# tfzhou/ContrastiveSeg

Hardware: AMD Instinct MI355X
Metric: images/sec contrastive train step, HRNet-W48 1024x512 bs8 (higher is better)
Workload: dtype fp32 in/out, f16x3 split MFMA (fp32 accumulate); 1 GPU; cfg2: BASELINE.json configs[1]: HRNet-W48 + contrast_ce_loss, synthetic Cityscapes 3x512x1024x19, tau=0.1, max_samples=1024, with_embed=True, SGD(0.01,0.9,5; model=hrnet_w48_contrast, loss=contrast_ce_loss, global_batch=8, per_gpu_batch=8, arithmetic=f16x3 on the matrix cores for the 3x3 / 1x1 convolutions, rest fp32, parallelism=dp1, step_graph=eager (auto: per-GPU batch above 1, the GPU is the limit)

## Files before the change

contrastiveseg_amd/_hip.py:

```python
import ctypes
import os

import torch

_PKG = os.path.dirname(os.path.abspath(__file__))
LIB_PATH = os.path.join(_PKG, "libcseg_hip.so")

_c_int = ctypes.c_int
_c_float = ctypes.c_float
_ptr = ctypes.c_void_p


class ContrastDesc(ctypes.Structure):
    _fields_ = [("mode", _c_int), ("N", _c_int), ("M", _c_int), ("D", _c_int),
                ("anchors", _ptr), ("a_lab", _ptr), ("contrast", _ptr), ("c_lab", _ptr),
                ("segment_queue", _ptr), ("pixel_queue", _ptr),
                ("bank_classes", _c_int), ("bank_size", _c_int),
                ("temperature", _c_float), ("base_temperature", _c_float)]


class ConvGroupMember(ctypes.Structure):
    _fields_ = [("x", _ptr), ("wp", _ptr), ("bias", _ptr), ("addend", _ptr), ("y", _ptr), ("stats", _ptr), ("amax_x", _ptr),
                ("amax_w", _ptr), ("B", _c_int), ("Cin", _c_int), ("Cout", _c_int), ("H", _c_int), ("W", _c_int),
                ("reserved", _c_int * 3)]
# ... 59 lines not shown
    "cseg_conv1x1_sb_packed_bytes": (ctypes.c_size_t, [_c_int, _c_int]),
    "cseg_conv1x1_sb_pack_weights": (_c_int, [_ptr, _c_int, _c_int, _c_int, _ptr, _ptr]),
    "cseg_conv1x1_sb_fwd": (_c_int, [_ptr, _ptr, _ptr, _c_int, _c_int, _c_int, _c_int, _ptr, _ptr]),
    "cseg_conv1x1_sb_wrw_ws_floats": (ctypes.c_size_t, [_c_int] * 4),
    "cseg_conv1x1_sb_wrw": (_c_int, [_ptr, _ptr, _c_int, _c_int, _c_int, _c_int, _ptr, _ptr, _ptr]),
    "cseg_amax_f32": (_c_int, [_ptr, ctypes.c_long, _ptr, _ptr]),
    "cseg_conv3x3_split_packed_bytes": (ctypes.c_size_t, [_c_int, _c_int, _c_int]),
    "cseg_conv3x3_split_pack": (_c_int, [_ptr, _c_int, _c_int, _c_int, _c_int, _c_int, _ptr, _ptr, _ptr]),
    "cseg_conv3x3_split_fwd": (_c_int, [_ptr, _ptr, _ptr] + [_c_int] * 7 + [_ptr, _ptr, _ptr, _ptr]),
    "cseg_conv3x3_split_wrw": (_c_int, [_ptr, _ptr] + [_c_int] * 6 + [_ptr, _ptr, _ptr, _ptr, _ptr]),
    "cseg_conv3x3_split_fwd_add": (_c_int, [_ptr, _ptr, _ptr, _ptr] + [_c_int] * 7 + [_ptr, _ptr, _ptr, _ptr]),
    "cseg_conv3x3_split_group_fwd": (_c_int, [_ptr, _c_int, _c_int, _ptr, _ptr]),
    "cseg_conv3x3_split_group_wrw": (_c_int, [_ptr, _c_int, _c_int, _ptr]),
    "cseg_bn_group_tiles_finalize": (_c_int, [_ptr, _c_int, _ptr]),
    "cseg_bn_group_apply": (_c_int, [_ptr, _c_int, _c_int, _ptr]),
    "cseg_bn_group_bwd": (_c_int, [_ptr, _c_int, _c_int, _c_int, _ptr]),
    "cseg_bn_group_tiles_moments": (_c_int, [_ptr, _c_int, _ptr, _ptr]),
    "cseg_bn_group_finalize": (_c_int, [_ptr, _c_int, _ptr, _ptr]),
    "cseg_bn_group_bwd_reduce": (_c_int, [_ptr, _c_int, _c_int, _ptr, _ptr]),
    "cseg_bn_group_bwd_apply": (_c_int, [_ptr, _c_int, _c_int, _ptr, _ptr]),
    "cseg_conv3x3_split_dil_fwd": (_c_int, [_ptr, _ptr, _ptr, _ptr] + [_c_int] * 7 + [_ptr, _ptr, _ptr, _ptr, _ptr]),
    "cseg_conv3x3_s2_split_packed_bytes": (ctypes.c_size_t, [_c_int] * 2),
    "cseg_conv3x3_s2_split_plan": (_c_int, [_c_int] * 4 + [_ptr, _ptr]),
    "cseg_conv3x3_s2_split_pack": (_c_int, [_ptr] + [_c_int] * 4 + [_ptr, _ptr, _ptr]),
    "cseg_conv3x3_s2_split_fwd": (_c_int, [_ptr, _ptr] + [_c_int] * 6 + [_ptr, _ptr, _ptr, _ptr]),
    "cseg_conv3x3_s2_split_bwd": (_c_int, [_ptr, _ptr] + [_c_int] * 6 + [_ptr, _ptr, _ptr, _ptr]),
    "cseg_conv3x3_s2_rgb_fwd": (_c_int, [_ptr, _ptr] + [_c_int] * 4 + [_ptr, _ptr]),
    "cseg_conv3x3_s2_rgb_wrw_ws_floats": (ctypes.c_size_t, [_c_int] * 4),
    "cseg_conv3x3_s2_rgb_wrw": (_c_int, [_ptr, _ptr] + [_c_int] * 4 + [_ptr, _ptr, _ptr]),
    "cseg_cls1x1_fwd": (_c_int, [_ptr, _ptr, _ptr] + [_c_int] * 4 + [ctypes.c_long, _ptr, _ptr]),
    "cseg_cls1x1_bwd": (_c_int, [_ptr, _ptr] + [_c_int] * 4 + [ctypes.c_long, _ptr, _ptr]),
    "cseg_cls1x1_wrw_ws_floats": (ctypes.c_size_t, [_c_int, _c_int, _c_int, ctypes.c_long]),
    "cseg_cls1x1_wrw": (_c_int, [_ptr, _ptr] + [_c_int] * 4 + [ctypes.c_long, _ptr, _ptr, _ptr]),
    "cseg_conv3x3_s2_wrw_ws_floats": (ctypes.c_size_t, [_c_int] * 5),
    "cseg_conv3x3_s2_split_wrw": (_c_int, [_ptr, _ptr] + [_c_int] * 6 + [_ptr, _ptr, _ptr, _ptr, _ptr]),
    "cseg_conv1x1_split_packed_bytes": (ctypes.c_size_t, [_c_int, _c_int, _c_int]),
    "cseg_conv1x1_split_pack": (_c_int, [_ptr, _c_int, _c_int, _c_int, _c_int, _ptr, _ptr, _ptr]),
    "cseg_conv1x1_split_fwd": (_c_int, [_ptr, _ptr, _ptr] + [_c_int] * 5 + [_ptr, _ptr, _ptr, _ptr]),
    "cseg_conv1x1_split_fwd_add": (_c_int, [_ptr, _ptr, _ptr, _ptr] + [_c_int] * 5 + [_ptr, _ptr, _ptr, _ptr]),
    "cseg_conv1x1_split_wrw": (_c_int, [_ptr, _ptr] + [_c_int] * 5 + [_ptr, _ptr, _ptr, _ptr, _ptr]),
    "cseg_conv3x3_split_plan": (_c_int, [_c_int, _c_int, _c_int, _ptr, _ptr, _ptr]),
    "cseg_conv1x1_split_plan": (_c_int, [_c_int, _c_int, _ptr, _ptr]),
    "cseg_conv1x1_split_plan_arith": (_c_int, [_c_int, _c_int, _c_int, ctypes.POINTER(_c_int), ctypes.POINTER(ctypes.c_long)]),
    "cseg_amax_batch": (_c_int, [_ptr, _c_int, _c_int, _ptr]),
    "cseg_split_pack_batch": (_c_int, [_ptr, _c_int, _c_int, _c_int, _ptr]),
    "cseg_augment_batch": (_c_int, [_ptr, _ptr, _ptr, _ptr] + [_c_int] * 5 + [_c_float, _ptr, _ptr, _ptr, _ptr, _ptr]),
    "cseg_conv_stat_segments": (ctypes.c_size_t, [_c_int] * 4),
    "cseg_conv3x3_split_fwd_st": (_c_int, [_ptr, _ptr, _ptr] + [_c_int] * 7 + [_ptr, _ptr, _ptr, _ptr, _ptr]),
    "cseg_conv1x1_split_fwd_st": (_c_int, [_ptr, _ptr, _ptr] + [_c_int] * 5 + [_ptr, _ptr, _ptr, _ptr, _ptr]),
    "cseg_conv3x3_s2_split_fwd_st": (_c_int, [_ptr, _ptr] + [_c_int] * 6 + [_ptr, _ptr, _ptr, _ptr, _ptr]),
    "cseg_bn_tiles_finalize": (_c_int, [_ptr, _c_int, ctypes.c_long, _c_float, _c_float, _ptr, _ptr, _ptr, _ptr, _ptr]),
    "cseg_bn_tiles_moments": (_c_int, [_ptr, _c_int, ctypes.c_long, _ptr, _ptr]),
    "cseg_bn_ws_floats": (ctypes.c_size_t, [_c_int, _c_int, _c_int]),
    "cseg_bn_stats": (_c_int, [_ptr, _c_int, _c_int, _c_int, _ptr, _ptr, _ptr]),
    "cseg_bn_finalize": (_c_int, [_ptr, _c_int, ctypes.c_double, _c_float, _c_float, _ptr, _ptr, _ptr, _ptr, _ptr]),
    "cseg_bn_stats_finalize": (_c_int, [_ptr, _c_int, _c_int, _c_int, _ptr, _c_float, _c_float, _ptr, _ptr, _ptr, _ptr,
                                        _ptr]),
    "cseg_bn_fwd": (_c_int, [_ptr] * 4 + [_c_int] * 4 + [_ptr, _c_float, _c_float] + [_ptr] * 5 + [_ptr]),
    "cseg_bn_bwd": (_c_int, [_ptr] * 6 + [_c_int] * 5 + [_ptr] * 5 + [_ptr]),
    "cseg_bn_fwd_amax": (_c_int, [_ptr] * 4 + [_c_int] * 4 + [_ptr, _c_float, _c_float] + [_ptr] * 5 + [_ptr, _ptr]),
    "cseg_bn_bwd_amax": (_c_int, [_ptr] * 6 + [_c_int] * 5 + [_ptr] * 5 + [_ptr, _ptr]),
    "cseg_bn_apply_amax": (_c_int, [_ptr, _ptr, _ptr, _ptr, _ptr, _c_int, _c_int, _c_int, _c_int, _ptr, _ptr, _ptr]),
    "cseg_bn_bwd_apply_amax": (_c_int, [_ptr] * 6 + [ctypes.c_double, _c_int, _c_int, _c_int, _c_int, _ptr, _ptr, _ptr]),
    "cseg_bn_apply": (_c_int, [_ptr, _ptr, _ptr, _ptr, _ptr, _c_int, _c_int, _c_int, _c_int, _ptr, _ptr]),
    "cseg_bn_bwd_reduce": (_c_int, [_ptr] * 6 + [_c_int] * 4 + [_ptr] * 5 + [_ptr]),
    "cseg_bn_bwd_apply": (_c_int, [_ptr] * 6 + [ctypes.c_double, _c_int, _c_int, _c_int, _c_int, _ptr, _ptr]),
# ... 54 lines not shown
```

contrastiveseg_amd/csrc/cls1x1.hip:

```cpp
#include "cseg_common.h"
#include "cseg_hip.h"

namespace {

constexpr int PX = 128;

template <int KP>
__global__ __launch_bounds__(256) void cls1x1_fwd_kernel(const float* __restrict__ x, const float* __restrict__ wt,
                                                         const float* __restrict__ bias, int C, int K, long P, int tiles,
                                                         float* __restrict__ y) {
    __shared__ float red[PX][KP + 1];
    const int b = blockIdx.x / tiles, tile = blockIdx.x - b * tiles;
    const int half = __builtin_amdgcn_readfirstlane((int)threadIdx.x / PX), lp = threadIdx.x - half * PX;
    const long p = (long)tile * PX + lp;
    const bool live = p < P;
    const long pc = live ? p : P - 1;
    const int c_mid = (C + 1) / 2;
    const int c0 = half ? c_mid : 0, c1 = half ? C : c_mid;
    const float* xp = x + ((size_t)b * C + c0) * P + pc;
    const float* wp = wt + ((size_t)b * C + c0) * KP;
    float acc[KP];
#pragma unroll
    for (int k = 0; k < KP; ++k) acc[k] = 0.f;
    int c = c0;
    for (; c + 8 <= c1; c += 8) {
        float v[8];
#pragma unroll
        for (int j = 0; j < 8; ++j) v[j] = xp[(size_t)j * P];
#pragma unroll
        for (int j = 0; j < 8; ++j)
#pragma unroll
            for (int k = 0; k < KP; ++k) acc[k] = __builtin_fmaf(v[j], wp[j * KP + k], acc[k]);
        xp += (size_t)8 * P;
        wp += 8 * KP;
    }
    for (; c < c1; ++c) {
        const float v = xp[0];
#pragma unroll
        for (int k = 0; k < KP; ++k) acc[k] = __builtin_fmaf(v, wp[k], acc[k]);
        xp += P;
        wp += KP;
    }
    if (half) {
#pragma unroll
        for (int k = 0; k < KP; ++k) red[lp][k] = acc[k];
    }
    __syncthreads();
    if (!half && live) {
        float* yp = y + (size_t)b * K * P + p;
#pragma unroll
        for (int k = 0; k < KP; ++k)
            if (k < K) yp[(size_t)k * P] = (acc[k] + red[lp][k]) + (bias ? bias[k] : 0.f);
    }
}

template <int KP, bool VEC>
__global__ __launch_bounds__(256) void cls1x1_bwd_kernel(const float* __restrict__ dy, const float* __restrict__ wt, int C, int K,
                                                         long P, int tiles, float* __restrict__ dx) {
    constexpr int V = VEC ? 4 : 1;
    const int b = blockIdx.x / tiles, tile = blockIdx.x - b * tiles;
    const long p = ((long)tile * 256 + threadIdx.x) * V;
    const bool live = p < P;
    const long pc = live ? p : 0;
    float d[KP][V];
#pragma unroll
    for (int k = 0; k < KP; ++k) {
        if (k < K) {
            const float* src = dy + ((size_t)b * K + k) * P + pc;
            if (VEC) {
                const float4 t4 = *reinterpret_cast<const float4*>(src);
                d[k][0] = t4.x; d[k][1 % V] = t4.y; d[k][2 % V] = t4.z; d[k][3 % V] = t4.w;
            } else {
                d[k][0] = *src;
            }
        } else {
#pragma unroll
            for (int t = 0; t < V; ++t) d[k][t] = 0.f;
        }
    }
    const int per = (C + (int)gridDim.y - 1) / (int)gridDim.y;
    const int c0 = blockIdx.y * per, c1 = min(C, c0 + per);
    const float* wp = wt + ((size_t)b * C + c0) * KP;
    float* op = dx + ((size_t)b * C + c0) * P + pc;
    for (int c = c0; c < c1; ++c) {
        float s[V];
#pragma unroll
        for (int t = 0; t < V; ++t) s[t] = 0.f;
#pragma unroll
        for (int k = 0; k < KP; ++k)
#pragma unroll
            for (int t = 0; t < V; ++t) s[t] = __builtin_fmaf(wp[k], d[k][t], s[t]);
        if (live) {
            if (VEC) *reinterpret_cast<float4*>(op) = make_float4(s[0], s[1 % V], s[2 % V], s[3 % V]);
            else *op = s[0];
        }
        wp += KP;
        op += P;
    }
}

constexpr int WC = 64, WP = 64;
constexpr int A_PITCH = WP + 1;

template <int KP, bool VEC>
__global__ __launch_bounds__(256) void cls1x1_wrw_kernel(const float* __restrict__ x, const float* __restrict__ dy, int C, int K, long P,
                                                         int c_tiles, int n_split, float* __restrict__ partial) {
    __shared__ __attribute__((aligned(16))) float As[WC * A_PITCH];
    __shared__ __attribute__((aligned(16))) float Ds[WP * KP];
    __shared__ float red[3][WC][KP + 1];
    int blk = blockIdx.x;
    const int split = blk % n_split; blk /= n_split;
    const int ct = blk % c_tiles;
    const int b = blk / c_tiles;
    const int tid = threadIdx.x, wave = tid >> 6, lane = tid & 63;
    const long stages = (P + WP - 1) / WP;
    const long s0 = stages * split / n_split, s1 = stages * (split + 1) / n_split;
    const int cb = ct * WC;
    float acc[KP];
#pragma unroll
    for (int k = 0; k < KP; ++k) acc[k] = 0.f;
    const int a_ch = tid >> 2, a_px = (tid & 3) * 16;
    const bool a_ok = cb + a_ch < C;
    const float* a_src = x + ((size_t)b * C + min(cb + a_ch, C - 1)) * P;
    const int d_k = tid >> 4, d_px = (tid & 15) * 4;
    for (long st = s0; st < s1; ++st) {
        const long p0 = st * WP;
        float av[16], dv0[4], dv1[4];
        if (VEC && p0 + WP <= P) {
#pragma unroll
            for (int q = 0; q < 4; ++q) {
                const float4 t4 = *reinterpret_cast<const float4*>(a_src + p0 + a_px + 4 * q);
                av[4 * q] = t4.x; av[4 * q + 1] = t4.y; av[4 * q + 2] = t4.z; av[4 * q + 3] = t4.w;
            }
        } else {
#pragma unroll
            for (int j = 0; j < 16; ++j) av[j] = p0 + a_px + j < P ? a_src[p0 + a_px + j] : 0.f;
        }
#pragma unroll
        for (int j = 0; j < 4; ++j) {
            const long p = p0 + d_px + j;
            dv0[j] = (d_k < K && p < P) ? dy[((size_t)b * K + d_k) * P + p] : 0.f;
            dv1[j] = (d_k + 16 < K && p < P) ? dy[((size_t)b * K + d_k + 16) * P + p] : 0.f;
        }
        __syncthreads();
#pragma unroll
        for (int j = 0; j < 16; ++j) As[a_ch * A_PITCH + a_px + j] = a_ok ? av[j] : 0.f;
#pragma unroll
        for (int j = 0; j < 4; ++j) {
            Ds[(d_px + j) * KP + d_k] = dv0[j];
            if (d_k + 16 < KP) Ds[(d_px + j) * KP + d_k + 16] = dv1[j];
        }
        __syncthreads();
#pragma unroll 4
        for (int j = 0; j < WP / 4; ++j) {
            const int p = wave * (WP / 4) + j;
            const float a = As[lane * A_PITCH + p];
#pragma unroll
            for (int k4 = 0; k4 < KP / 4; ++k4) {
                const float4 d4 = *reinterpret_cast<const float4*>(Ds + p * KP + 4 * k4);
                acc[4 * k4] = __builtin_fmaf(a, d4.x, acc[4 * k4]);
                acc[4 * k4 + 1] = __builtin_fmaf(a, d4.y, acc[4 * k4 + 1]);
                acc[4 * k4 + 2] = __builtin_fmaf(a, d4.z, acc[4 * k4 + 2]);
                acc[4 * k4 + 3] = __builtin_fmaf(a, d4.w, acc[4 * k4 + 3]);
            }
        }
    }
    if (wave > 0) {
#pragma unroll
        for (int k = 0; k < KP; ++k) red[wave - 1][lane][k] = acc[k];
    }
    __syncthreads();
    if (wave == 0 && cb + lane < C) {
        const int B = gridDim.x / (n_split * c_tiles);
        float* out = partial + (((size_t)split * B + b) * C + (cb + lane)) * KP;
#pragma unroll
        for (int k = 0; k < KP; ++k) out[k] = ((acc[k] + red[0][lane][k]) + red[1][lane][k]) + red[2][lane][k];
    }
}

__global__ __launch_bounds__(256) void cls1x1_wrw_reduce_kernel(const float* __restrict__ partial, int n_split, long total,
                                                                float* __restrict__ dwt) {
    const long e = (long)blockIdx.x * 256 + threadIdx.x;
    if (e >= total) return;
    float s = 0.f;
    for (int sp = 0; sp < n_split; ++sp) s += partial[(size_t)sp * total + e];
    dwt[e] = s;
}

int wrw_splits(int B, int C, long P) {
    const long stages = (P + WP - 1) / WP;
    const long groups = (long)B * ((C + WC - 1) / WC);
    long n = (1536 + groups - 1) / groups;
    if (n > stages) n = stages;
    if (n > 64) n = 64;
    return (int)(n < 1 ? 1 : n);
}

bool shape_ok(int B, int C, int K, int KP, long P) {
    return B > 0 && C > 0 && K > 0 && K <= KP && (KP == 20 || KP == 32) && P > 0 && (long)B * C * P < (1L << 40) &&
           (long)B * ((P + PX - 1) / PX) < 2147483647L / 16;
}

}

extern "C" int cseg_cls1x1_fwd(const float* x, const float* wt, const float* bias, int B, int C, int K, int KP, long P, float* y,
                               cseg_stream_t stream_) {
    CSEG_REQUIRE(x && wt && y, "cls1x1_fwd: null pointer");
    CSEG_REQUIRE(shape_ok(B, C, K, KP, P), "cls1x1_fwd: unsupported shape B=%d C=%d K=%d KP=%d P=%ld (K <= KP, KP 20 or 32)", B, C, K, KP, P);
    hipStream_t stream = (hipStream_t)stream_;
    const int tiles = (int)((P + PX - 1) / PX);
    if (KP == 20)
        hipLaunchKernelGGL(cls1x1_fwd_kernel<20>, dim3((unsigned)(B * tiles)), dim3(256), 0, stream, x, wt, bias, C, K, P, tiles, y);
    else
        hipLaunchKernelGGL(cls1x1_fwd_kernel<32>, dim3((unsigned)(B * tiles)), dim3(256), 0, stream, x, wt, bias, C, K, P, tiles, y);
    CSEG_CHECK_LAUNCH("cls1x1_fwd_kernel");
    return 1;
}

extern "C" int cseg_cls1x1_bwd(const float* dy, const float* wt, int B, int C, int K, int KP, long P, float* dx, cseg_stream_t stream_) {
    CSEG_REQUIRE(dy && wt && dx, "cls1x1_bwd: null pointer");
    CSEG_REQUIRE(shape_ok(B, C, K, KP, P), "cls1x1_bwd: unsupported shape B=%d C=%d K=%d KP=%d P=%ld (K <= KP, KP 20 or 32)", B, C, K, KP, P);
    hipStream_t stream = (hipStream_t)stream_;
    const bool vec = P % 4 == 0 && ((reinterpret_cast<uintptr_t>(dy) | reinterpret_cast<uintptr_t>(dx)) & 15) == 0;
    const long per_block = vec ? 1024 : 256;
    const int tiles = (int)((P + per_block - 1) / per_block);
    int parts = 1;
    while (parts < 16 && (long)B * tiles * parts < 2048 && C / (parts * 2) >= 32) parts *= 2;
#define CLS_BWD(KPV, V)                                                                                                                \
    hipLaunchKernelGGL((cls1x1_bwd_kernel<KPV, V>), dim3((unsigned)(B * tiles), parts), dim3(256), 0, stream, dy, wt, C, K, P, tiles, dx)
    if (KP == 20) { if (vec) CLS_BWD(20, true); else CLS_BWD(20, false); }
    else          { if (vec) CLS_BWD(32, true); else CLS_BWD(32, false); }
#undef CLS_BWD
    CSEG_CHECK_LAUNCH("cls1x1_bwd_kernel");
    return 1;
}

extern "C" size_t cseg_cls1x1_wrw_ws_floats(int B, int C, int KP, long P) {
    if (B <= 0 || C <= 0 || P <= 0 || (KP != 20 && KP != 32)) return 0;
    return (size_t)wrw_splits(B, C, P) * B * C * KP;
}

extern "C" int cseg_cls1x1_wrw(const float* x, const float* dy, int B, int C, int K, int KP, long P, float* ws, float* dwt,
                               cseg_stream_t stream_) {
    CSEG_REQUIRE(x && dy && ws && dwt, "cls1x1_wrw: null pointer");
    CSEG_REQUIRE(shape_ok(B, C, K, KP, P), "cls1x1_wrw: unsupported shape B=%d C=%d K=%d KP=%d P=%ld (K <= KP, KP 20 or 32)", B, C, K, KP, P);
    hipStream_t stream = (hipStream_t)stream_;
    const int n_split = wrw_splits(B, C, P), c_tiles = (C + WC - 1) / WC;
    const long blocks = (long)B * c_tiles * n_split;
    CSEG_REQUIRE(blocks < 2147483647L, "cls1x1_wrw: grid too large");
    const bool vec = P % 4 == 0 && (reinterpret_cast<uintptr_t>(x) & 15) == 0;
#define CLS_WRW(KPV, V)                                                                                                            \
    hipLaunchKernelGGL((cls1x1_wrw_kernel<KPV, V>), dim3((unsigned)blocks), dim3(256), 0, stream, x, dy, C, K, P, c_tiles, n_split, ws)
    if (KP == 20) { if (vec) CLS_WRW(20, true); else CLS_WRW(20, false); }
    else          { if (vec) CLS_WRW(32, true); else CLS_WRW(32, false); }
#undef CLS_WRW
    CSEG_CHECK_LAUNCH("cls1x1_wrw_kernel");
    const long total = (long)B * C * KP;
    hipLaunchKernelGGL(cls1x1_wrw_reduce_kernel, dim3((unsigned)((total + 255) / 256)), dim3(256), 0, stream, ws, n_split, total, dwt);
    CSEG_CHECK_LAUNCH("cls1x1_wrw_reduce_kernel");
    return 1;
}
```

contrastiveseg_amd/kernels.py:

```python
import ctypes

import os

import torch
from torch.autograd import Function

from . import _hip

I32, I16, I64, F32 = torch.int32, torch.int16, torch.int64, torch.float32


def _p(t, dtype, what):
    return _hip.dev(t, dtype, what)


def _null():
    return ctypes.c_void_p(None)


def _on_device(t):
    return t.is_cuda


def _pq(t, what):
# ... 1826 lines not shown
        K_, KP, P = ctx.K, wt.shape[2], H * W
        dx = dwt = db = None
        if ctx.needs_input_grad[0]:
            dx = torch.empty_like(x)
            _hip.call("cseg_cls1x1_bwd", _p(dy, F32, "dy"), _p(wt, F32, "wt"), B, C, K_, KP, ctypes.c_long(P), _pf(dx), _hip.stream_ptr())
        if ctx.needs_input_grad[1]:
            n = _hip.lib().cseg_cls1x1_wrw_ws_floats(B, C, KP, ctypes.c_long(P))
            if n == 0:
                raise RuntimeError("cls1x1_wrw: unsupported shape %s x %s" % (tuple(x.shape), tuple(dy.shape)))
            ws = torch.empty(n, dtype=F32, device=x.device)
            dwt = torch.empty(B, C, KP, dtype=F32, device=x.device)
            _hip.call("cseg_cls1x1_wrw", _p(x, F32, "x"), _p(dy, F32, "dy"), B, C, K_, KP, ctypes.c_long(P), _pf(ws), _pf(dwt),
                      _hip.stream_ptr())
        if ctx.has_bias and ctx.needs_input_grad[2]:
            db = dy.sum((0, 2, 3))
        return dx, dwt, db, None


def cls1x1_weights(weight, B, mask=None):
    K_, C = weight.shape[:2]
    KP = cls1x1_kp(K_)
    w2 = weight.reshape(K_, C).t()
    if KP > K_:
        w2 = torch.nn.functional.pad(w2, (0, KP - K_))
    if mask is None:
        return w2.unsqueeze(0).expand(B, C, KP).contiguous()
    return w2.unsqueeze(0) * mask.reshape(B, C, 1)


def cls1x1(x, weight, bias=None, mask=None):
    return Cls1x1.apply(x, cls1x1_weights(weight, x.shape[0], mask), bias, weight.shape[0])


CONV1X1_SPLIT_BF16 = os.environ.get("CSEG_CONV1X1_SPLIT_BF16", "1") == "1"
CONV1X1_SB_MIN_TILES = int(os.environ.get("CSEG_SB_MIN_TILES", "1"))


def conv1x1_sb_eligible(x, weight):
    if not (_on_device(x) and x.dtype == F32 and weight.dtype == F32 and x.dim() == 4 and x.is_contiguous()):
        return False
    co, ci, kh, kw = weight.shape
    ok = lambda c: c % 48 == 0 or c % 64 == 0
    return (kh, kw) == (1, 1) and ok(ci) and ok(co) and x.shape[1] == ci


def conv1x1_sb_tiles(x, c_out):
    nt16 = next(16 * nt for nt in (9, 8, 6, 4, 3) if c_out % (16 * nt) == 0)
    return x.shape[0] * (c_out // nt16) * ((x.shape[2] * x.shape[3] + 255) // 256)


def conv1x1_sb_pack(weight, transpose=False):
    return SPLIT_WEIGHTS.get(weight, "c1", transpose, 0)


def conv1x1_sb_run(x, weight, transpose=False, bias=None, ax=None, want_stats=False, addend=None):
    co, ci = weight.shape[:2]
    conv_in, conv_out = (co, ci) if transpose else (ci, co)
    B, _, H, W = x.shape
    arith = split_arith_id()
    wp, aw = conv1x1_sb_pack(weight, transpose)
    if arith and ax is None:
        ax = tensor_amax(x)
    y = torch.empty(B, conv_out, H, W, dtype=F32, device=x.device)
    if want_stats and CONV_EPILOGUE_STATS:
        st = tile_stats_buffer(1, conv_out, B, H * W, 1, x.device)
        _hip.call("cseg_conv1x1_split_fwd_st", _pq(x, "x"), wp.data_ptr(), _opt(bias, F32, "bias"), B, conv_in, conv_out, H * W,
# ... 168 lines not shown
```

contrastiveseg_amd/lib/models/nets/hrnet.py:

```python
import torch
import torch.nn as nn

from contrastiveseg_amd import kernels as K
from contrastiveseg_amd.lib.models.backbones.backbone_selector import BackboneSelector
from contrastiveseg_amd.lib.models.modules.projection import ProjectionHead
from contrastiveseg_amd.lib.models.modules.spatial_ocr_block import SpatialGather_Module, SpatialOCR_Module
from contrastiveseg_amd.lib.models.tools.module_helper import (ClassifierConv1x1, FoldedDropout2d, HeadConv3x3, ModuleHelper,
                                                                  SplitConv2d)


import os as _os

_HEAD_STREAMS = {}
HEAD_FORK = _os.environ.get("CSEG_HEAD_FORK", "0") == "1"


def _fork_heads(feats):
    from contrastiveseg_amd.lib.models.backbones import hrnet_backbone as HB
    if not (HEAD_FORK and feats.is_cuda and HB.EAGER_FORKS and torch.is_grad_enabled()) or torch.cuda.is_current_stream_capturing():
        return None
    key = feats.device.index
    if key not in _HEAD_STREAMS:
        _HEAD_STREAMS[key] = torch.cuda.Stream(device=feats.device)
    return torch.cuda.current_stream(feats.device), _HEAD_STREAMS[key]


class HRNet_W48_CONTRAST(nn.Module):
    def __init__(self, configer):
        super(HRNet_W48_CONTRAST, self).__init__()
        self.configer = configer
        self.num_classes = self.configer.get('data', 'num_classes')
        self.backbone = BackboneSelector(configer).get_backbone()
        self.proj_dim = self.configer.get('contrast', 'proj_dim')
        in_channels = self.backbone.num_features
        conv3x3 = HeadConv3x3(in_channels)
        bnrelu = ModuleHelper.BNReLU(in_channels, bn_type=self.configer.get('network', 'bn_type'))
        classifier = ClassifierConv1x1(in_channels, self.num_classes, kernel_size=1, stride=1, padding=0, bias=False)
        self.cls_head = nn.Sequential(conv3x3, bnrelu, FoldedDropout2d(0.10, classifier), classifier)
        self.proj_head = ProjectionHead(dim_in=in_channels, proj_dim=self.proj_dim)

    def forward(self, x_, with_embed=False, is_eval=False):
        feats = K.upsample_concat(self.backbone(x_))
        fork = _fork_heads(feats)
        if fork is not None:
            cur, side = fork
            side.wait_stream(cur)
            feats.record_stream(side)
            with torch.cuda.stream(side):
                emb = self.proj_head(feats)
        out = {'seg': self.cls_head(feats)}
        if out['seg'].is_cuda and self.training and not torch.cuda.is_current_stream_capturing():
            out['seg_ready'] = torch.cuda.Event()
            out['seg_ready'].record()
        if fork is not None:
            cur.wait_stream(side)
            emb.record_stream(cur)
            out['embed'] = emb
        else:
            out['embed'] = self.proj_head(feats)
        return out


class HRNet_W48_OCR_CONTRAST(nn.Module):
    def __init__(self, configer):
        super(HRNet_W48_OCR_CONTRAST, self).__init__()
        self.configer = configer
        self.num_classes = self.configer.get('data', 'num_classes')
        self.backbone = BackboneSelector(configer).get_backbone()
        self.proj_dim = self.configer.get('contrast', 'proj_dim')
        bn_type = self.configer.get('network', 'bn_type')
        in_channels = self.backbone.num_features
# ... 61 lines not shown
```

include/cseg_hip.h:

```cpp
#ifndef CSEG_HIP_H
#define CSEG_HIP_H

#include <stddef.h>
#include <stdint.h>

#ifdef __cplusplus
extern "C" {
#endif

typedef void* cseg_stream_t;

int cseg_abi_version(void);
const char* cseg_last_error(void);

int cseg_classify_partition(const float* seg, const int64_t* pred_in, const int64_t* target, int B, int K, int h, int w, int H, int W,
                            int ignore_label, int32_t* lab, int32_t* pred, int16_t* key, int32_t* counts,
                            int32_t* seg_off, int32_t* part_idx, int32_t* status, cseg_stream_t stream);

int cseg_gather_anchors(const float* embed, int B, int D, int P, const int32_t* part_idx,
                        const int32_t* sel_pos, int N, float* anchors, int32_t* sel_pix, cseg_stream_t stream);

int cseg_scatter_anchor_grad(const float* d_anchor_parts, int n_parts, const int32_t* sel_pix, int N, int D,
                             int P, float scale, float* d_embed, cseg_stream_t stream);

// ... 228 lines not shown
#define CSEG_PACK_C1 2
#define CSEG_PACK_C3_S2T 3
int cseg_conv3x3_split_plan(int conv_in, int conv_out, int nt_request, int* kind, int* nt, long* threads);
int cseg_conv1x1_split_plan(int conv_in, int conv_out, int* nt, long* threads);
int cseg_conv1x1_split_plan_arith(int arith, int conv_in, int conv_out, int* nt, long* threads);
typedef struct cseg_split_job {
    const void* src;
    void* dst;
    unsigned* amax;
    int cout, cin, flag, nt, kind, total, block0, reserved;
} cseg_split_job;
int cseg_amax_batch(const cseg_split_job* jobs_dev, int n_jobs, int total_blocks, cseg_stream_t stream);
int cseg_split_pack_batch(const cseg_split_job* jobs_dev, int n_jobs, int total_blocks, int arith, cseg_stream_t stream);
size_t cseg_conv1x1_split_packed_bytes(int arith, int Cin, int Cout);
int cseg_conv1x1_split_pack(const float* w, int Cout, int Cin, int transpose, int arith, const unsigned* amax_w, void* wp,
                            cseg_stream_t stream);
int cseg_conv1x1_split_fwd(const float* x, const void* wp, const float* bias, int B, int Cin, int Cout, int HW, int arith,
                           const unsigned* amax_x, const unsigned* amax_w, float* y, cseg_stream_t stream);
int cseg_conv1x1_split_fwd_add(const float* x, const void* wp, const float* bias, const float* addend, int B, int Cin, int Cout, int HW,
                               int arith, const unsigned* amax_x, const unsigned* amax_w, float* y, cseg_stream_t stream);
int cseg_conv1x1_split_wrw(const float* x, const float* dy, int B, int Cin, int Cout, int HW, int arith, const unsigned* amax_x,
                           const unsigned* amax_dy, float* ws, float* dw, cseg_stream_t stream);

int cseg_conv3x3_s2_rgb_fwd(const float* x, const float* w, int B, int Cout, int H, int W, float* y, cseg_stream_t stream);
size_t cseg_conv3x3_s2_rgb_wrw_ws_floats(int B, int Cout, int H, int W);
int cseg_conv3x3_s2_rgb_wrw(const float* x, const float* dy, int B, int Cout, int H, int W, float* ws, float* dw, cseg_stream_t stream);

int cseg_cls1x1_fwd(const float* x, const float* wt, const float* bias, int B, int C, int K, int KP, long P, float* y,
                    cseg_stream_t stream);
int cseg_cls1x1_bwd(const float* dy, const float* wt, int B, int C, int K, int KP, long P, float* dx, cseg_stream_t stream);
size_t cseg_cls1x1_wrw_ws_floats(int B, int C, int KP, long P);
int cseg_cls1x1_wrw(const float* x, const float* dy, int B, int C, int K, int KP, long P, float* ws, float* dwt, cseg_stream_t stream);

#define CSEG_AUG_PARAM_INTS 12
int cseg_augment_batch(const uint8_t* img, const uint8_t* lab, const int16_t* lut, const int32_t* params, int B, int Hs,
                       int Ws, int Ht, int Wt, float div_value, const float* mean3, const float* std3, float* out_img,
                       int64_t* out_lab, cseg_stream_t stream);

#ifdef __cplusplus
}
#endif
#endif
```

Baseline: 97.42 images/sec.

## Fold classifier-head BatchNorm+ReLU into the 1x1 classifier forward and backward kernels

Adds a ClassifierHead path that applies BN normalization and ReLU on the fly inside the cls1x1 forward and weight-gradient kernels, using precomputed tile statistics instead of a separate BN-ReLU output tensor. A new fused backward computes the ReLU-masked classifier input gradient, reduces the BN gradient sums per channel and applies the BN backward in one more pass, so the BN-ReLU activation tensor is never written or re-read. It is enabled by default through an environment flag. The cost is recomputing the BN-ReLU transform in several kernels, a smaller unroll in the fused forward, and more kernel-code complexity.

```diff
diff --git a/contrastiveseg_amd/_hip.py b/contrastiveseg_amd/_hip.py
--- a/contrastiveseg_amd/_hip.py
+++ b/contrastiveseg_amd/_hip.py
@@ -115,6 +115,10 @@
     "cseg_cls1x1_bwd": (_c_int, [_ptr, _ptr] + [_c_int] * 4 + [ctypes.c_long, _ptr, _ptr]),
     "cseg_cls1x1_wrw_ws_floats": (ctypes.c_size_t, [_c_int, _c_int, _c_int, ctypes.c_long]),
     "cseg_cls1x1_wrw": (_c_int, [_ptr, _ptr] + [_c_int] * 4 + [ctypes.c_long, _ptr, _ptr, _ptr]),
+    "cseg_cls1x1_bn_fwd": (_c_int, [_ptr] * 6 + [_c_int] * 4 + [ctypes.c_long, _ptr, _ptr]),
+    "cseg_cls1x1_bn_wrw": (_c_int, [_ptr] * 5 + [_c_int] * 4 + [ctypes.c_long, _ptr, _ptr, _ptr]),
+    "cseg_cls1x1_bn_bwd_ws_floats": (ctypes.c_size_t, [_c_int, _c_int, _c_int, ctypes.c_long]),
+    "cseg_cls1x1_bn_bwd": (_c_int, [_ptr] * 6 + [_c_int] * 4 + [ctypes.c_long] + [_ptr] * 6),
     "cseg_conv3x3_s2_wrw_ws_floats": (ctypes.c_size_t, [_c_int] * 5),
     "cseg_conv3x3_s2_split_wrw": (_c_int, [_ptr, _ptr] + [_c_int] * 6 + [_ptr, _ptr, _ptr, _ptr, _ptr]),
     "cseg_conv1x1_split_packed_bytes": (ctypes.c_size_t, [_c_int, _c_int, _c_int]),
diff --git a/contrastiveseg_amd/csrc/cls1x1.hip b/contrastiveseg_amd/csrc/cls1x1.hip
--- a/contrastiveseg_amd/csrc/cls1x1.hip
+++ b/contrastiveseg_amd/csrc/cls1x1.hip
@@ -1,12 +1,26 @@
-#include "cseg_common.h"
-#include "cseg_hip.h"
+#include "cseg_split.h"
 
 namespace {
 
 constexpr int PX = 128;
 
-template <int KP>
-__global__ __launch_bounds__(256) void cls1x1_fwd_kernel(const float* __restrict__ x, const float* __restrict__ wt,
+struct ClsBn {
+    const float* mean_invstd;
+    const float* gamma;
+    const float* beta;
+};
+struct ClsBnCh {
+    float mean = 0.f, a = 1.f, beta = 0.f;
+    __device__ __forceinline__ ClsBnCh() {}
+    __device__ __forceinline__ ClsBnCh(const ClsBn& bn, int c)
+        : mean(bn.mean_invstd[2 * c]), a((bn.gamma ? bn.gamma[c] : 1.f) * bn.mean_invstd[2 * c + 1]), beta(bn.beta ? bn.beta[c] : 0.f) {}
+    __device__ __forceinline__ float operator()(float v) const {
+        return __builtin_elementwise_maximum(fmaf(v - mean, a, beta), 0.f);
+    }
+};
+
+template <int KP, bool BN>
+__global__ __launch_bounds__(256) void cls1x1_fwd_kernel(const float* __restrict__ x, const ClsBn bn, const float* __restrict__ wt,
                                                          const float* __restrict__ bias, int C, int K, long P, int tiles,
                                                          float* __restrict__ y) {
     __shared__ float red[PX][KP + 1];
@@ -22,20 +36,25 @@
     float acc[KP];
 #pragma unroll
     for (int k = 0; k < KP; ++k) acc[k] = 0.f;
+    constexpr int U = BN ? 4 : 8;
     int c = c0;
-    for (; c + 8 <= c1; c += 8) {
-        float v[8];
-#pragma unroll
-        for (int j = 0; j < 8; ++j) v[j] = xp[(size_t)j * P];
-#pragma unroll
-        for (int j = 0; j < 8; ++j)
+    for (; c + U <= c1; c += U) {
+        float v[U];
+#pragma unroll
+        for (int j = 0; j < U; ++j) v[j] = xp[(size_t)j * P];
+        if (BN) {
+#pragma unroll
+            for (int j = 0; j < U; ++j) v[j] = ClsBnCh(bn, c + j)(v[j]);
+        }
+#pragma unroll
+        for (int j = 0; j < U; ++j)
 #pragma unroll
             for (int k = 0; k < KP; ++k) acc[k] = __builtin_fmaf(v[j], wp[j * KP + k], acc[k]);
-        xp += (size_t)8 * P;
-        wp += 8 * KP;
+        xp += (size_t)U * P;
+        wp += U * KP;
     }
     for (; c < c1; ++c) {
-        const float v = xp[0];
+        const float v = BN ? ClsBnCh(bn, c)(xp[0]) : xp[0];
 #pragma unroll
         for (int k = 0; k < KP; ++k) acc[k] = __builtin_fmaf(v, wp[k], acc[k]);
         xp += P;
@@ -102,9 +121,9 @@
 constexpr int WC = 64, WP = 64;
 constexpr int A_PITCH = WP + 1;
 
-template <int KP, bool VEC>
-__global__ __launch_bounds__(256) void cls1x1_wrw_kernel(const float* __restrict__ x, const float* __restrict__ dy, int C, int K, long P,
-                                                         int c_tiles, int n_split, float* __restrict__ partial) {
+template <int KP, bool VEC, bool BN>
+__global__ __launch_bounds__(256) void cls1x1_wrw_kernel(const float* __restrict__ x, const ClsBn bn, const float* __restrict__ dy, int C,
+                                                         int K, long P, int c_tiles, int n_split, float* __restrict__ partial) {
     __shared__ __attribute__((aligned(16))) float As[WC * A_PITCH];
     __shared__ __attribute__((aligned(16))) float Ds[WP * KP];
     __shared__ float red[3][WC][KP + 1];
@@ -122,6 +141,8 @@
     const int a_ch = tid >> 2, a_px = (tid & 3) * 16;
     const bool a_ok = cb + a_ch < C;
     const float* a_src = x + ((size_t)b * C + min(cb + a_ch, C - 1)) * P;
+    ClsBnCh act;
+    if (BN) act = ClsBnCh(bn, min(cb + a_ch, C - 1));
     const int d_k = tid >> 4, d_px = (tid & 15) * 4;
     for (long st = s0; st < s1; ++st) {
         const long p0 = st * WP;
@@ -132,9 +153,13 @@
                 const float4 t4 = *reinterpret_cast<const float4*>(a_src + p0 + a_px + 4 * q);
                 av[4 * q] = t4.x; av[4 * q + 1] = t4.y; av[4 * q + 2] = t4.z; av[4 * q + 3] = t4.w;
             }
+            if (BN) {
+#pragma unroll
+                for (int j = 0; j < 16; ++j) av[j] = act(av[j]);
+            }
         } else {
 #pragma unroll
-            for (int j = 0; j < 16; ++j) av[j] = p0 + a_px + j < P ? a_src[p0 + a_px + j] : 0.f;
+            for (int j = 0; j < 16; ++j) av[j] = p0 + a_px + j < P ? (BN ? act(a_src[p0 + a_px + j]) : a_src[p0 + a_px + j]) : 0.f;
         }
 #pragma unroll
         for (int j = 0; j < 4; ++j) {
@@ -187,6 +212,175 @@
     dwt[e] = s;
 }
 
+typedef float f32x2 __attribute__((ext_vector_type(2)));
+constexpr int BN_PART_MAX = 512;
+
+template <bool VEC>
+__device__ __forceinline__ void cls_load_px(const float* __restrict__ src, float (&v)[VEC ? 4 : 1]) {
+    constexpr int V = VEC ? 4 : 1;
+    if (VEC) {
+        const float4 t4 = *reinterpret_cast<const float4*>(src);
+        v[0] = t4.x; v[1 % V] = t4.y; v[2 % V] = t4.z; v[3 % V] = t4.w;
+    } else {
+        v[0] = *src;
+    }
+}
+
+template <int KP, bool VEC>
+__device__ __forceinline__ void cls_masked_dz(const float* __restrict__ wp, const float (&d)[KP][VEC ? 4 : 1], const ClsBnCh ch, bool live,
+                                              float (&xv)[VEC ? 4 : 1], float (&s)[VEC ? 4 : 1]) {
+    constexpr int V = VEC ? 4 : 1;
+    if (VEC) {
+        f32x2 sa = {0.f, 0.f}, sb = {0.f, 0.f};
+#pragma unroll
+        for (int k = 0; k < KP; ++k) {
+            const f32x2 w2 = {wp[k], wp[k]};
+            sa = __builtin_elementwise_fma(w2, f32x2{d[k][0], d[k][1 % V]}, sa);
+            sb = __builtin_elementwise_fma(w2, f32x2{d[k][2 % V], d[k][3 % V]}, sb);
+        }
+        s[0] = sa.x; s[1 % V] = sa.y; s[2 % V] = sb.x; s[3 % V] = sb.y;
+    } else {
+        s[0] = 0.f;
+#pragma unroll
+        for (int k = 0; k < KP; ++k) s[0] = __builtin_fmaf(wp[k], d[k][0], s[0]);
+    }
+#pragma unroll
+    for (int t = 0; t < V; ++t) {
+        xv[t] = live ? xv[t] - ch.mean : 0.f;
+        s[t] = fmaf(xv[t], ch.a, ch.beta) > 0.f ? s[t] : 0.f;
+    }
+}
+
+template <int KP, bool VEC, bool APPLY>
+__global__ __launch_bounds__(256) void cls1x1_bn_bwd_kernel(const float* __restrict__ g, const float* __restrict__ wt,
+                                                            const float* __restrict__ cx, const ClsBn bn, const float* __restrict__ coef,
+                                                            int C, int K, long P, int tiles, float* __restrict__ partial,
+                                                            float* __restrict__ dc, unsigned* __restrict__ amax_out) {
+    constexpr int V = VEC ? 4 : 1;
+    __shared__ float red[APPLY ? 1 : BN_PART_MAX][4][2];
+    const int b = blockIdx.x / tiles, tile = blockIdx.x - b * tiles;
+    const long p = ((long)tile * 256 + threadIdx.x) * V;
+    const bool live = p < P;
+    const long pc = live ? p : 0;
+    float d[KP][V];
+#pragma unroll
+    for (int k = 0; k < KP; ++k) {
+        if (k < K && live) {
+            const float* src = g + ((size_t)b * K + k) * P + pc;
+            if (VEC) {
+                const float4 t4 = *reinterpret_cast<const float4*>(src);
+                d[k][0] = t4.x; d[k][1 % V] = t4.y; d[k][2 % V] = t4.z; d[k][3 % V] = t4.w;
+            } else {
+                d[k][0] = *src;
+            }
+        } else {
+#pragma unroll
+            for (int t = 0; t < V; ++t) d[k][t] = 0.f;
+        }
+    }
+    const int per = (C + (int)gridDim.y - 1) / (int)gridDim.y;
+    const int c0 = blockIdx.y * per, c1 = min(C, c0 + per);
+    const float* wp = wt + ((size_t)b * C + c0) * KP;
+    const float* xp = cx + ((size_t)b * C + c0) * P + pc;
+    float* op = APPLY ? dc + ((size_t)b * C + c0) * P + pc : nullptr;
+    unsigned am = 0;
+    if constexpr (APPLY) {
+        for (int c = c0; c < c1; ++c) {
+            float s[V], xv[V];
+            cls_load_px<VEC>(xp, xv);
+            cls_masked_dz<KP, VEC>(wp, d, ClsBnCh(bn, c), live, xv, s);
+            const float a = ClsBnCh(bn, c).a, k0 = coef[4 * c], k0l = coef[4 * c + 1], k1 = coef[4 * c + 2];
+            float o[V];
+#pragma unroll
+            for (int t = 0; t < V; ++t) {
+                o[t] = a * ((s[t] - k0) - k0l - xv[t] * k1);
+                if (live) am = max(am, __builtin_bit_cast(unsigned, o[t]) & 0x7fffffffu);
+            }
+            if (live) {
+                if (VEC) *reinterpret_cast<float4*>(op) = make_float4(o[0], o[1 % V], o[2 % V], o[3 % V]);
+                else *op = o[0];
+            }
+            op += P;
+            wp += KP;
+            xp += P;
+        }
+    } else {
+        float nx[V];
+        if (c0 < c1) cls_load_px<VEC>(xp, nx);
+        for (int c = c0; c < c1; ++c) {
+            float s[V], xv[V];
+#pragma unroll
+            for (int t = 0; t < V; ++t) xv[t] = nx[t];
+            xp += P;
+            if (c + 1 < c1) cls_load_px<VEC>(xp, nx);
+            cls_masked_dz<KP, VEC>(wp, d, ClsBnCh(bn, c), live, xv, s);
+            float s0, s1;
+            if (VEC) {
+                s0 = (s[0] + s[1 % V]) + (s[2 % V] + s[3 % V]);
+                s1 = (s[0] * xv[0] + s[1 % V] * xv[1 % V]) + (s[2 % V] * xv[2 % V] + s[3 % V] * xv[3 % V]);
+            } else {
+                s0 = s[0];
+                s1 = s[0] * xv[0];
+            }
+            s0 = wave_sum(s0);
+            s1 = wave_sum(s1);
+            if ((threadIdx.x & 63) == 0) { red[c - c0][threadIdx.x >> 6][0] = s0; red[c - c0][threadIdx.x >> 6][1] = s1; }
+            wp += KP;
+        }
+    }
+    if (APPLY) {
+        if (amax_out) {
+#pragma unroll
+            for (int o = 32; o > 0; o >>= 1) am = max(am, (unsigned)__shfl_xor((int)am, o, 64));
+            amax_publish_waves(am, amax_out);
+        }
+    } else {
+        __syncthreads();
+        float* out = partial + ((size_t)blockIdx.x * C + c0) * 2;
+        for (int i = threadIdx.x; i < (c1 - c0) * 2; i += 256) {
+            const int cl = i >> 1, j = i & 1;
+            out[i] = (red[cl][0][j] + red[cl][1][j]) + (red[cl][2][j] + red[cl][3][j]);
+        }
+    }
+}
+
+__global__ __launch_bounds__(256) void cls1x1_bn_sums_kernel(const float* __restrict__ partial, int S, int C, double inv_count,
+                                                             const float* __restrict__ mean_invstd, float* __restrict__ coef,
+                                                             float* __restrict__ d_gamma, float* __restrict__ d_beta) {
+    const int c = blockIdx.x * 4 + (threadIdx.x >> 6), lane = threadIdx.x & 63;
+    if (c >= C) return;
+    double s0 = 0.0, s1 = 0.0;
+    for (int s = lane; s < S; s += 64) {
+        s0 += (double)partial[((size_t)s * C + c) * 2 + 0];
+        s1 += (double)partial[((size_t)s * C + c) * 2 + 1];
+    }
+#pragma unroll
+    for (int o = 32; o > 0; o >>= 1) { s0 += __shfl_xor(s0, o, 64); s1 += __shfl_xor(s1, o, 64); }
+    if (lane == 0) {
+        const double invstd = (double)mean_invstd[2 * c + 1];
+        const double k0d = s0 * inv_count;
+        const float k0 = (float)k0d;
+        coef[4 * c] = k0;
+        coef[4 * c + 1] = (float)(k0d - (double)k0);
+        coef[4 * c + 2] = (float)(s1 * inv_count * invstd * invstd);
+        coef[4 * c + 3] = 0.f;
+        if (d_gamma) d_gamma[c] = (float)(s1 * invstd);
+        if (d_beta) d_beta[c] = (float)s0;
+    }
+}
+
+struct BnBwdPlan { bool vec; int tiles, parts; };
+BnBwdPlan bn_bwd_plan(int B, int C, long P, bool aligned) {
+    BnBwdPlan pl;
+    pl.vec = P % 4 == 0 && aligned;
+    const long per_block = pl.vec ? 1024 : 256;
+    pl.tiles = (int)((P + per_block - 1) / per_block);
+    pl.parts = 1;
+    while (pl.parts < 16 && (long)B * pl.tiles * pl.parts < 2048 && C / (pl.parts * 2) >= 32) pl.parts *= 2;
+    while ((C + pl.parts - 1) / pl.parts > BN_PART_MAX) pl.parts *= 2;
+    return pl;
+}
+
 int wrw_splits(int B, int C, long P) {
     const long stages = (P + WP - 1) / WP;
     const long groups = (long)B * ((C + WC - 1) / WC);
@@ -209,11 +403,27 @@
     CSEG_REQUIRE(shape_ok(B, C, K, KP, P), "cls1x1_fwd: unsupported shape B=%d C=%d K=%d KP=%d P=%ld (K <= KP, KP 20 or 32)", B, C, K, KP, P);
     hipStream_t stream = (hipStream_t)stream_;
     const int tiles = (int)((P + PX - 1) / PX);
+    const ClsBn bn = {nullptr, nullptr, nullptr};
     if (KP == 20)
-        hipLaunchKernelGGL(cls1x1_fwd_kernel<20>, dim3((unsigned)(B * tiles)), dim3(256), 0, stream, x, wt, bias, C, K, P, tiles, y);
+        hipLaunchKernelGGL((cls1x1_fwd_kernel<20, false>), dim3((unsigned)(B * tiles)), dim3(256), 0, stream, x, bn, wt, bias, C, K, P, tiles, y);
     else
-        hipLaunchKernelGGL(cls1x1_fwd_kernel<32>, dim3((unsigned)(B * tiles)), dim3(256), 0, stream, x, wt, bias, C, K, P, tiles, y);
+        hipLaunchKernelGGL((cls1x1_fwd_kernel<32, false>), dim3((unsigned)(B * tiles)), dim3(256), 0, stream, x, bn, wt, bias, C, K, P, tiles, y);
     CSEG_CHECK_LAUNCH("cls1x1_fwd_kernel");
+    return 1;
+}
+
+extern "C" int cseg_cls1x1_bn_fwd(const float* x, const float* mean_invstd, const float* gamma, const float* beta, const float* wt,
+                                  const float* bias, int B, int C, int K, int KP, long P, float* y, cseg_stream_t stream_) {
+    CSEG_REQUIRE(x && mean_invstd && wt && y, "cls1x1_bn_fwd: null pointer");
+    CSEG_REQUIRE(shape_ok(B, C, K, KP, P), "cls1x1_bn_fwd: unsupported shape B=%d C=%d K=%d KP=%d P=%ld (K <= KP, KP 20 or 32)", B, C, K, KP, P);
+    hipStream_t stream = (hipStream_t)stream_;
+    const int tiles = (int)((P + PX - 1) / PX);
+    const ClsBn bn = {mean_invstd, gamma, beta};
+    if (KP == 20)
+        hipLaunchKernelGGL((cls1x1_fwd_kernel<20, true>), dim3((unsigned)(B * tiles)), dim3(256), 0, stream, x, bn, wt, bias, C, K, P, tiles, y);
+    else
+        hipLaunchKernelGGL((cls1x1_fwd_kernel<32, true>), dim3((unsigned)(B * tiles)), dim3(256), 0, stream, x, bn, wt, bias, C, K, P, tiles, y);
+    CSEG_CHECK_LAUNCH("cls1x1_bn_fwd_kernel");
     return 1;
 }
 
@@ -240,19 +450,22 @@
     return (size_t)wrw_splits(B, C, P) * B * C * KP;
 }
 
-extern "C" int cseg_cls1x1_wrw(const float* x, const float* dy, int B, int C, int K, int KP, long P, float* ws, float* dwt,
-                               cseg_stream_t stream_) {
-    CSEG_REQUIRE(x && dy && ws && dwt, "cls1x1_wrw: null pointer");
-    CSEG_REQUIRE(shape_ok(B, C, K, KP, P), "cls1x1_wrw: unsupported shape B=%d C=%d K=%d KP=%d P=%ld (K <= KP, KP 20 or 32)", B, C, K, KP, P);
+static int cls1x1_wrw_impl(const char* who, const float* x, const ClsBn bn, const float* dy, int B, int C, int K, int KP, long P, float* ws,
+                           float* dwt, cseg_stream_t stream_) {
+    CSEG_REQUIRE(x && dy && ws && dwt, "%s: null pointer", who);
+    CSEG_REQUIRE(shape_ok(B, C, K, KP, P), "%s: unsupported shape B=%d C=%d K=%d KP=%d P=%ld (K <= KP, KP 20 or 32)", who, B, C, K, KP, P);
     hipStream_t stream = (hipStream_t)stream_;
     const int n_split = wrw_splits(B, C, P), c_tiles = (C + WC - 1) / WC;
     const long blocks = (long)B * c_tiles * n_split;
-    CSEG_REQUIRE(blocks < 2147483647L, "cls1x1_wrw: grid too large");
+    CSEG_REQUIRE(blocks < 2147483647L, "%s: grid too large", who);
     const bool vec = P % 4 == 0 && (reinterpret_cast<uintptr_t>(x) & 15) == 0;
-#define CLS_WRW(KPV, V)                                                                                                            \
-    hipLaunchKernelGGL((cls1x1_wrw_kernel<KPV, V>), dim3((unsigned)blocks), dim3(256), 0, stream, x, dy, C, K, P, c_tiles, n_split, ws)
-    if (KP == 20) { if (vec) CLS_WRW(20, true); else CLS_WRW(20, false); }
-    else          { if (vec) CLS_WRW(32, true); else CLS_WRW(32, false); }
+    const bool fold = bn.mean_invstd != nullptr;
+#define CLS_WRW(KPV, V, F)                                                                                                         \
+    hipLaunchKernelGGL((cls1x1_wrw_kernel<KPV, V, F>), dim3((unsigned)blocks), dim3(256), 0, stream, x, bn, dy, C, K, P, c_tiles, n_split, ws)
+#define CLS_WRW_V(KPV, V) do { if (fold) CLS_WRW(KPV, V, true); else CLS_WRW(KPV, V, false); } while (0)
+    if (KP == 20) { if (vec) CLS_WRW_V(20, true); else CLS_WRW_V(20, false); }
+    else          { if (vec) CLS_WRW_V(32, true); else CLS_WRW_V(32, false); }
+#undef CLS_WRW_V
 #undef CLS_WRW
     CSEG_CHECK_LAUNCH("cls1x1_wrw_kernel");
     const long total = (long)B * C * KP;
@@ -260,3 +473,51 @@
     CSEG_CHECK_LAUNCH("cls1x1_wrw_reduce_kernel");
     return 1;
 }
+
+extern "C" int cseg_cls1x1_wrw(const float* x, const float* dy, int B, int C, int K, int KP, long P, float* ws, float* dwt,
+                               cseg_stream_t stream_) {
+    return cls1x1_wrw_impl("cls1x1_wrw", x, ClsBn{nullptr, nullptr, nullptr}, dy, B, C, K, KP, P, ws, dwt, stream_);
+}
+
+extern "C" int cseg_cls1x1_bn_wrw(const float* x, const float* mean_invstd, const float* gamma, const float* beta, const float* dy, int B,
+                                  int C, int K, int KP, long P, float* ws, float* dwt, cseg_stream_t stream_) {
+    CSEG_REQUIRE(mean_invstd, "cls1x1_bn_wrw: null pointer");
+    return cls1x1_wrw_impl("cls1x1_bn_wrw", x, ClsBn{mean_invstd, gamma, beta}, dy, B, C, K, KP, P, ws, dwt, stream_);
+}
+
+extern "C" size_t cseg_cls1x1_bn_bwd_ws_floats(int B, int C, int KP, long P) {
+    if (B <= 0 || C <= 0 || P <= 0 || (KP != 20 && KP != 32)) return 0;
+    const long tiles = (P + 255) / 256;
+    return (size_t)B * tiles * C * 2 + (size_t)C * 4;
+}
+
+extern "C" int cseg_cls1x1_bn_bwd(const float* g, const float* wt, const float* x, const float* mean_invstd, const float* gamma,
+                                  const float* beta, int B, int C, int K, int KP, long P, float* ws, float* d_gamma, float* d_beta,
+                                  float* dx, unsigned* amax_out, cseg_stream_t stream_) {
+    CSEG_REQUIRE(g && wt && x && mean_invstd && ws, "cls1x1_bn_bwd: null pointer");
+    CSEG_REQUIRE(shape_ok(B, C, K, KP, P), "cls1x1_bn_bwd: unsupported shape B=%d C=%d K=%d KP=%d P=%ld (K <= KP, KP 20 or 32)", B, C, K, KP, P);
+    hipStream_t stream = (hipStream_t)stream_;
+    const bool aligned = ((reinterpret_cast<uintptr_t>(g) | reinterpret_cast<uintptr_t>(x) | reinterpret_cast<uintptr_t>(dx)) & 15) == 0;
+    const BnBwdPlan pl = bn_bwd_plan(B, C, P, aligned);
+    CSEG_REQUIRE((C + pl.parts - 1) / pl.parts <= BN_PART_MAX && pl.parts <= 65535, "cls1x1_bn_bwd: too many channels (%d)", C);
+    const int S = B * pl.tiles;
+    float* coef = ws + (size_t)S * C * 2;
+    const ClsBn bn = {mean_invstd, gamma, beta};
+    const dim3 grid((unsigned)S, (unsigned)pl.parts);
+#define CLS_BNB(KPV, V, A)                                                                                                      \
+    hipLaunchKernelGGL((cls1x1_bn_bwd_kernel<KPV, V, A>), grid, dim3(256), 0, stream, g, wt, x, bn, coef, C, K, P, pl.tiles, ws, dx, amax_out)
+#define CLS_BNB_V(A) do { if (KP == 20) { if (pl.vec) CLS_BNB(20, true, A); else CLS_BNB(20, false, A); }                        \
+                          else          { if (pl.vec) CLS_BNB(32, true, A); else CLS_BNB(32, false, A); } } while (0)
+    CLS_BNB_V(false);
+    CSEG_CHECK_LAUNCH("cls1x1_bn_bwd_kernel (reduce)");
+    hipLaunchKernelGGL(cls1x1_bn_sums_kernel, dim3((unsigned)((C + 3) / 4)), dim3(256), 0, stream, ws, S, C,
+                       1.0 / ((double)B * (double)P), mean_invstd, coef, d_gamma, d_beta);
+    CSEG_CHECK_LAUNCH("cls1x1_bn_sums_kernel");
+    if (dx) {
+        CLS_BNB_V(true);
+        CSEG_CHECK_LAUNCH("cls1x1_bn_bwd_kernel (apply)");
+    }
+#undef CLS_BNB_V
+#undef CLS_BNB
+    return 1;
+}
diff --git a/contrastiveseg_amd/kernels.py b/contrastiveseg_amd/kernels.py
--- a/contrastiveseg_amd/kernels.py
+++ b/contrastiveseg_amd/kernels.py
@@ -1882,6 +1882,71 @@
     return Cls1x1.apply(x, cls1x1_weights(weight, x.shape[0], mask), bias, weight.shape[0])
 
 
+CLS_BN_FOLD = os.environ.get("CSEG_CLS_BN_FOLD", "1") == "1"
+
+
+class ClsHeadBN(Function):
+
+    @staticmethod
+    def forward(ctx, y, gamma, beta, running_mean, running_var, num_batches_tracked, momentum, eps, wt, bias, K_):
+        wt = wt.contiguous()
+        B, C, H, W = y.shape
+        KP = wt.shape[2]
+        mi = bn_tiles_finalize(known_tile_stats(y), eps, momentum, running_mean, running_var, num_batches_tracked)
+        seg = torch.empty(B, K_, H, W, dtype=F32, device=y.device)
+        _hip.call("cseg_cls1x1_bn_fwd", _p(y, F32, "y"), _pf(mi), _opt(gamma, F32, "weight"), _opt(beta, F32, "bias"), _p(wt, F32, "wt"),
+                  _opt(bias, F32, "bias"), B, C, K_, KP, ctypes.c_long(H * W), _pf(seg), _hip.stream_ptr())
+        ctx.save_for_backward(y, mi, gamma, beta, wt)
+        ctx.K = K_
+        ctx.has_bias = bias is not None
+        return seg
+
+    @staticmethod
+    def backward(ctx, g):
+        y, mi, gamma, beta, wt = ctx.saved_tensors
+        g = g.contiguous()
+        B, C, H, W = y.shape
+        K_, KP, P = ctx.K, wt.shape[2], H * W
+        dev = y.device
+        lib = _hip.lib()
+        dwt = db = None
+        if ctx.needs_input_grad[8]:
+            n = lib.cseg_cls1x1_wrw_ws_floats(B, C, KP, ctypes.c_long(P))
+            if n == 0:
+                raise RuntimeError("cls1x1_bn_wrw: unsupported shape %s x %s" % (tuple(y.shape), tuple(g.shape)))
+            ws = torch.empty(n, dtype=F32, device=dev)
+            dwt = torch.empty(B, C, KP, dtype=F32, device=dev)
+            _hip.call("cseg_cls1x1_bn_wrw", _pf(y), _pf(mi), _opt(gamma, F32, "weight"), _opt(beta, F32, "bias"), _p(g, F32, "dy"),
+                      B, C, K_, KP, ctypes.c_long(P), _pf(ws), _pf(dwt), _hip.stream_ptr())
+        n = lib.cseg_cls1x1_bn_bwd_ws_floats(B, C, KP, ctypes.c_long(P))
+        if n == 0:
+            raise RuntimeError("cls1x1_bn_bwd: unsupported shape %s x %s" % (tuple(y.shape), tuple(g.shape)))
+        ws = torch.empty(n, dtype=F32, device=dev)
+        d_wb = torch.empty(2, C, dtype=F32, device=dev)
+        dy = torch.empty_like(y) if ctx.needs_input_grad[0] else None
+        amax = amax_request(y) if dy is not None else None
+        _hip.call("cseg_cls1x1_bn_bwd", _p(g, F32, "dy"), _pf(wt), _pf(y), _pf(mi), _opt(gamma, F32, "weight"), _opt(beta, F32, "bias"),
+                  B, C, K_, KP, ctypes.c_long(P), _pf(ws), _pf(d_wb[0]), _pf(d_wb[1]), _pf(dy) if dy is not None else _null(),
+                  _pf(amax) if amax is not None else _null(), _hip.stream_ptr())
+        if dy is not None:
+            amax_attach(dy, amax)
+            mark_zero_channel_sum(dy)
+        if ctx.has_bias and ctx.needs_input_grad[9]:
+            db = g.sum((0, 2, 3))
+        return (dy, d_wb[0] if gamma is not None else None, d_wb[1] if beta is not None else None, None, None, None, None, None,
+                dwt, db, None)
+
+
+def cls_head_bn_eligible(y, bn_weight, cls_weight):
+    return (CLS_BN_FOLD and cls1x1_eligible(y, cls_weight) and y.is_contiguous() and known_tile_stats(y) is not None
+            and bn_weight is not None and bn_weight.dtype == F32)
+
+
+def cls_head_bn(y, bn, weight, bias=None, mask=None):
+    return ClsHeadBN.apply(y, bn.weight, bn.bias, bn.running_mean, bn.running_var, bn.num_batches_tracked, float(bn.momentum),
+                           float(bn.eps), cls1x1_weights(weight, y.shape[0], mask), bias, weight.shape[0])
+
+
 CONV1X1_SPLIT_BF16 = os.environ.get("CSEG_CONV1X1_SPLIT_BF16", "1") == "1"
 CONV1X1_SB_MIN_TILES = int(os.environ.get("CSEG_SB_MIN_TILES", "1"))
 
diff --git a/contrastiveseg_amd/lib/models/nets/hrnet.py b/contrastiveseg_amd/lib/models/nets/hrnet.py
--- a/contrastiveseg_amd/lib/models/nets/hrnet.py
+++ b/contrastiveseg_amd/lib/models/nets/hrnet.py
@@ -5,8 +5,8 @@
 from contrastiveseg_amd.lib.models.backbones.backbone_selector import BackboneSelector
 from contrastiveseg_amd.lib.models.modules.projection import ProjectionHead
 from contrastiveseg_amd.lib.models.modules.spatial_ocr_block import SpatialGather_Module, SpatialOCR_Module
-from contrastiveseg_amd.lib.models.tools.module_helper import (ClassifierConv1x1, FoldedDropout2d, HeadConv3x3, ModuleHelper,
-                                                                  SplitConv2d)
+from contrastiveseg_amd.lib.models.tools.module_helper import (ClassifierConv1x1, ClassifierHead, FoldedDropout2d, HeadConv3x3,
+                                                                  ModuleHelper, SplitConv2d)
 
 
 import os as _os
@@ -36,7 +36,7 @@
         conv3x3 = HeadConv3x3(in_channels)
         bnrelu = ModuleHelper.BNReLU(in_channels, bn_type=self.configer.get('network', 'bn_type'))
         classifier = ClassifierConv1x1(in_channels, self.num_classes, kernel_size=1, stride=1, padding=0, bias=False)
-        self.cls_head = nn.Sequential(conv3x3, bnrelu, FoldedDropout2d(0.10, classifier), classifier)
+        self.cls_head = ClassifierHead(conv3x3, bnrelu, FoldedDropout2d(0.10, classifier), classifier)
         self.proj_head = ProjectionHead(dim_in=in_channels, proj_dim=self.proj_dim)
 
     def forward(self, x_, with_embed=False, is_eval=False):
diff --git a/include/cseg_hip.h b/include/cseg_hip.h
--- a/include/cseg_hip.h
+++ b/include/cseg_hip.h
@@ -284,6 +284,15 @@
 size_t cseg_cls1x1_wrw_ws_floats(int B, int C, int KP, long P);
 int cseg_cls1x1_wrw(const float* x, const float* dy, int B, int C, int K, int KP, long P, float* ws, float* dwt, cseg_stream_t stream);
 
+int cseg_cls1x1_bn_fwd(const float* x, const float* mean_invstd, const float* gamma, const float* beta, const float* wt,
+                       const float* bias, int B, int C, int K, int KP, long P, float* y, cseg_stream_t stream);
+int cseg_cls1x1_bn_wrw(const float* x, const float* mean_invstd, const float* gamma, const float* beta, const float* dy, int B, int C,
+                       int K, int KP, long P, float* ws, float* dwt, cseg_stream_t stream);
+size_t cseg_cls1x1_bn_bwd_ws_floats(int B, int C, int KP, long P);
+int cseg_cls1x1_bn_bwd(const float* g, const float* wt, const float* x, const float* mean_invstd, const float* gamma, const float* beta,
+                       int B, int C, int K, int KP, long P, float* ws, float* d_gamma, float* d_beta, float* dx, unsigned* amax_out,
+                       cseg_stream_t stream);
+
 #define CSEG_AUG_PARAM_INTS 12
 int cseg_augment_batch(const uint8_t* img, const uint8_t* lab, const int16_t* lut, const int32_t* params, int B, int Hs,
                        int Ws, int Ht, int Wt, float div_value, const float* mean3, const float* std3, float* out_img,
```

Result: slower. 95.49 images/sec (-2.0%).
